# Project-MONAI/GenerativeModels

Hardware: NVIDIA H100
Metric: ddim50_voxels_per_s (higher is better)
Workload: dtype fp16

## Files before the change

generativemodels_b200/_lib.py:

```python
from __future__ import annotations

import ctypes as C
import os
from pathlib import Path

_HERE = Path(__file__).resolve().parent
ACT_DTYPE = os.environ.get("B200_ACT_DTYPE", "fp16").lower()
if ACT_DTYPE in ("float16", "half", "f16"):
    ACT_DTYPE = "fp16"
if ACT_DTYPE in ("bfloat16",):
    ACT_DTYPE = "bf16"
if ACT_DTYPE not in ("fp16", "bf16"):
    raise ValueError(f"B200_ACT_DTYPE must be fp16 or bf16, got {ACT_DTYPE!r}")
LIB_PATH = _HERE / "lib" / ("libb200gen.so" if ACT_DTYPE == "fp16" else "libb200gen_bf16.so")

B200_OK, B200_EINVAL, B200_ENOTSUP, B200_ECUDA, B200_ENODEV = 0, -1, -2, -3, -4
DT_H16, DT_F32 = 0, 1
DT_F64, DT_FP16, DT_BF16 = 2, 3, 4
SSIM_MAX_K, SSIM_MAX_SCALES = 128, 32
H16_FP16, H16_BF16 = 0, 1
ACT_NONE, ACT_RELU, ACT_SILU, ACT_LEAKYRELU, ACT_GELU, ACT_TANH, ACT_SIGMOID = 0, 1, 2, 3, 4, 5, 6
ACT_GEGLU = 7
ACT_LEAKYRELU02 = 8
INTERP_BILINEAR, INTERP_BICUBIC = 0, 1
POOL_AVG, POOL_MAX = 0, 1
(INTERPOLATE_NEAREST, INTERPOLATE_LINEAR, INTERPOLATE_BILINEAR, INTERPOLATE_BICUBIC, INTERPOLATE_TRILINEAR,
 INTERPOLATE_AREA) = 0, 1, 2, 3, 4, 5
PRED_EPSILON, PRED_SAMPLE, PRED_V = 0, 1, 2
IGEMM_MAX_SEG = 128


class B200Error(RuntimeError):
    pass


class IgemmSeg(C.Structure):
    _fields_ = [("src", C.c_int8), ("dw", C.c_int8), ("dh", C.c_int8), ("dd", C.c_int8),
                ("c0", C.c_uint16), ("nchunks", C.c_uint16)]


class IgemmParams(C.Structure):
    _fields_ = [
        ("a_ptr", C.c_void_p * 2), ("a_C", C.c_int32 * 2), ("a_pitch", C.c_int32 * 2),
        ("in_N", C.c_int32), ("in_D", C.c_int32), ("in_H", C.c_int32), ("in_W", C.c_int32),
        ("stride_d", C.c_int32), ("stride_h", C.c_int32), ("stride_w", C.c_int32),
        ("w_ptr", C.c_void_p), ("w_rows", C.c_int32), ("w_pitch", C.c_int32), ("w_K", C.c_int32),
        ("w_bstride", C.c_int64), ("w_batched", C.c_int32), ("n_seg", C.c_int32),
        ("seg", IgemmSeg * IGEMM_MAX_SEG),
        ("out_ptr", C.c_void_p), ("out_dtype", C.c_int32),
        ("out_N", C.c_int32), ("out_D", C.c_int32), ("out_H", C.c_int32), ("out_W", C.c_int32),
        ("cout", C.c_int32), ("out_cols", C.c_int32),
        ("out_sN", C.c_int64), ("out_sD", C.c_int64), ("out_sH", C.c_int64), ("out_sW", C.c_int64),
        ("bias", C.c_void_p), ("rowvec", C.c_void_p), ("rowvec_bstride", C.c_int64), ("row_bias", C.c_void_p),
        ("act1", C.c_int32), ("scale", C.c_float),
        ("res_ptr", C.c_void_p), ("res_dtype", C.c_int32),
        ("res_sN", C.c_int64), ("res_sD", C.c_int64), ("res_sH", C.c_int64), ("res_sW", C.c_int64),
        ("act2", C.c_int32), ("stat_ptr", C.c_void_p), ("impl", C.c_int32),
        ("gn_partial", C.c_void_p), ("gn_slots", C.c_int32), ("gn_slot0", C.c_int32),
        ("split_ws", C.c_void_p), ("split_ws_bytes", C.c_int64),
        ("a_broadcast", C.c_int32), ("gn_group", C.c_int32),
    ]


class GnStatsParams(C.Structure):
    _fields_ = [("x_ptr", C.c_void_p * 2), ("x_C", C.c_int32 * 2), ("x_pitch", C.c_int32 * 2),
                ("N", C.c_int32), ("spatial", C.c_int64), ("groups", C.c_int32), ("eps", C.c_float),
                ("gamma", C.c_void_p), ("beta", C.c_void_p), ("partial", C.c_void_p), ("affine", C.c_void_p)]


class GnApplyParams(C.Structure):
    _fields_ = [("x_ptr", C.c_void_p * 2), ("x_C", C.c_int32 * 2), ("x_pitch", C.c_int32 * 2),
                ("N", C.c_int32), ("spatial", C.c_int64), ("affine", C.c_void_p), ("act", C.c_int32),
                ("y_ptr", C.c_void_p), ("y_pitch", C.c_int32)]


class FlashParams(C.Structure):
    _fields_ = [("q", C.c_void_p), ("k", C.c_void_p), ("vt", C.c_void_p), ("out", C.c_void_p), ("res", C.c_void_p),
                ("B", C.c_int32), ("T", C.c_int32), ("S", C.c_int32), ("heads", C.c_int32), ("dh", C.c_int32),
                ("q_pitch", C.c_int32), ("k_pitch", C.c_int32), ("vt_pitch", C.c_int32), ("out_pitch", C.c_int32),
                ("res_pitch", C.c_int32), ("scale", C.c_float),
                ("workspace", C.c_void_p), ("workspace_bytes", C.c_int64)]


class DdimCoef(C.Structure):
    _fields_ = [("sqrt_alpha_prod_t", C.c_float), ("sqrt_beta_prod_t", C.c_float),
                ("sqrt_alpha_prod_prev", C.c_float), ("dir_coef", C.c_float), ("sigma", C.c_float),
                ("clip_min", C.c_float), ("clip_max", C.c_float),
                ("prediction_type", C.c_int32), ("clip", C.c_int32)]


class DdpmCoef(C.Structure):
    _fields_ = [("sqrt_alpha_prod_t", C.c_float), ("sqrt_beta_prod_t", C.c_float),
                ("coef_x0", C.c_float), ("coef_xt", C.c_float), ("sigma", C.c_float),
                ("clip_min", C.c_float), ("clip_max", C.c_float), ("min_log", C.c_float), ("max_log", C.c_float),
                ("var_mode", C.c_int32), ("prediction_type", C.c_int32), ("clip", C.c_int32)]

# ... 156 lines not shown
```

generativemodels_b200/csrc/igemm.cu:

```cuda
#include "common.cuh"
#include "wgmma.cuh"
#include <cuda.h>
#include <cudaTypedefs.h>
#include <mutex>
#include <string.h>

namespace b200 {

static constexpr int kBM = 128;
static constexpr int kBK = 64;
static constexpr int kABytes = kBM * kBK * 2;
static constexpr int kMmaWarp0 = 4;
static constexpr int kTmaWarp = 12;
static constexpr int kThreads = 13 * 32;

struct SegDev {
  int8_t src, dw, dh, dd;
  uint16_t c0, nchunks;
};

struct IgemmDev {
  alignas(64) CUtensorMap tmA[2];
  alignas(64) CUtensorMap tmB;
  const h16* a_ptr[2];
  int a_C[2], a_pitch[2];
  int in_N, in_D, in_H, in_W;
  int a_bcast;
  const h16* w_ptr;
  int w_rows, w_K, w_pitch;
  long long w_bstride;
  int w_batched;
  int n_seg, num_k_chunks;
  int sd, sh, sw;
  int N, OD, OH, OW;
  int BW, BH, BD, bw_log2, bh_log2;
  int tiles_w, tiles_h, tiles_d, tiles_n, num_tiles;
  int k_splits;
  long long split_stride;
  void* out_ptr;
  int out_dtype, cout, out_cols, out_vec, out_staged, out_v256;
  float* stat_ptr;
  float* gn_partial;
  int gn_slots, gn_slot0;
  int gn_sh;
  long long out_sN, out_sD, out_sH, out_sW;
  const float* bias;
  const float* rowvec;
  long long rowvec_bstride;
  const float* row_bias;
  int act1, act2;
  int geglu;
  float scale;
  const void* res_ptr;
  int res_dtype, res_vec, res_v256;
  long long res_sN, res_sD, res_sH, res_sW;
  SegDev seg[B200_IGEMM_MAX_SEG];
};

__device__ __forceinline__ void tma_load_5d(const CUtensorMap* tm, uint32_t bar, uint32_t dst, int c0,
                                            int c1, int c2, int c3, int c4) {
  asm volatile(
      "cp.async.bulk.tensor.5d.shared::cluster.global.mbarrier::complete_tx::bytes"
      " [%0], [%1, {%3, %4, %5, %6, %7}], [%2];" ::"r"(dst),
      "l"(reinterpret_cast<uint64_t>(tm)), "r"(bar), "r"(c0), "r"(c1), "r"(c2), "r"(c3), "r"(c4)
      : "memory");
}
template <int CH>
__device__ __forceinline__ void acc_ld(const float* src, uint32_t* r) {
#pragma unroll
  for (int j = 0; j < CH; j += 4) {
    const float4 t = *reinterpret_cast<const float4*>(src + j);
    r[j] = __float_as_uint(t.x); r[j + 1] = __float_as_uint(t.y);
    r[j + 2] = __float_as_uint(t.z); r[j + 3] = __float_as_uint(t.w);
  }
}

__host__ __device__ __forceinline__ int split_begin(int num_k, int splits, int ks) {
  return (int)(((long long)num_k * ks) / splits);
// ... 1145 lines not shown
  B200_CUDA(rc);
  if (max_clusters < 1) { set_error("igemm: no cluster of igemm_wide_kernel fits on this device"); return B200_ECUDA; }
  const int clusters = d.num_tiles < max_clusters ? d.num_tiles : max_clusters;
  B200_CUDA(b200::launch_kernel<wide::kCluster>(igemm_wide_kernel, clusters * wide::kCluster, wide::kThreads,
                                                wide::kSmem, stream, d));
  B200_LAUNCH_CHECK("igemm_wide_kernel");
  return B200_OK;
}

}

using namespace b200;

extern "C" int64_t b200_igemm_split_workspace_bytes(const b200_igemm_params* p) {
  if (!p || p->n_seg < 1 || p->n_seg > B200_IGEMM_MAX_SEG || p->out_N < 1 || p->out_D < 1 || p->out_H < 1 ||
      p->out_W < 1 || p->out_cols < 1 || p->stride_d < 1 || p->stride_h < 1 || p->stride_w < 1)
    return 0;
  if (p->impl == 1) return 0;
  return make_plan(p, true).ws_bytes;
}

extern "C" int b200_igemm_plan(const b200_igemm_params* p, int32_t sm_count_, int32_t with_workspace, int32_t out[4]) {
  if (!p || !out || sm_count_ < 1 || p->n_seg < 1 || p->n_seg > B200_IGEMM_MAX_SEG || p->out_N < 1 || p->out_D < 1 ||
      p->out_H < 1 || p->out_W < 1 || p->out_cols < 1)
    return B200_EINVAL;
  const Plan pl = make_plan(p, with_workspace != 0, sm_count_);
  out[0] = pl.BN;
  out[1] = pl.splits;
  out[2] = (int32_t)pl.ntiles;
  out[3] = 0;
  return B200_OK;
}

extern "C" int b200_igemm(const b200_igemm_params* p, void* stream_v) {
  cudaStream_t stream = static_cast<cudaStream_t>(stream_v);
  B200_CHECK_ARG(p != nullptr, "igemm: null params");
  B200_CHECK_ARG(p->a_ptr[0] && p->w_ptr && p->out_ptr, "igemm: null tensor pointer");
  B200_CHECK_ARG(p->n_seg >= 1 && p->n_seg <= B200_IGEMM_MAX_SEG, "igemm: n_seg=%d out of range", p->n_seg);
  B200_CHECK_ARG(p->in_N >= 1 && p->in_D >= 1 && p->in_H >= 1 && p->in_W >= 1, "igemm: bad input extent");
  B200_CHECK_ARG(p->out_N == p->in_N && p->out_D >= 1 && p->out_H >= 1 && p->out_W >= 1, "igemm: bad output extent");
  const bool geglu = p->act1 == B200_ACT_GEGLU;
  B200_CHECK_ARG(p->cout >= 1 && p->out_cols >= (geglu ? p->cout / 2 : p->cout), "igemm: bad cout/out_cols");
  if (geglu) {
    B200_CHECK_ARG(p->cout % 64 == 0 && p->out_cols == p->cout / 2 && p->out_dtype == B200_DT_H16 && !p->res_ptr &&
                   p->scale == 1.0f && p->act2 == B200_ACT_NONE && !p->stat_ptr && !p->gn_partial && !p->row_bias &&
                   p->impl != 1,
                   "igemm: B200_ACT_GEGLU needs cout %% 64 == 0, out_cols == cout / 2, a h16 output and no residual / "
                   "scale / act2 / statistics / row bias (and has no cross-check kernel)");
  }
  B200_CHECK_ARG(p->w_pitch % 8 == 0 && p->w_rows >= 1, "igemm: weight pitch must be a multiple of 8");
  B200_CHECK_ARG(((uintptr_t)p->w_ptr & 15) == 0, "igemm: weight pointer not 16-byte aligned");
  B200_CHECK_ARG(p->stride_d >= 1 && p->stride_d <= 8 && p->stride_h >= 1 && p->stride_h <= 8 &&
                 p->stride_w >= 1 && p->stride_w <= 8, "igemm: stride out of range");
  for (int s = 0; s < 2; ++s) {
    if (!p->a_ptr[s]) continue;
    B200_CHECK_ARG(p->a_pitch[s] % 8 == 0 && p->a_C[s] >= 1 && p->a_C[s] <= p->a_pitch[s],
                   "igemm: source %d channel pitch %d / extent %d invalid", s, p->a_pitch[s], p->a_C[s]);
    B200_CHECK_ARG(((uintptr_t)p->a_ptr[s] & 15) == 0, "igemm: source %d not 16-byte aligned", s);
  }
  std::call_once(g_encode_once, load_encode);
  if (!g_encode) { set_error("igemm: cuTensorMapEncodeTiled entry point unavailable"); return B200_ECUDA; }

  IgemmDev d;
  memset(&d, 0, sizeof(d));
  int kchunks = 0;
  for (int s = 0; s < p->n_seg; ++s) {
    const b200_igemm_seg& sg = p->seg[s];
    B200_CHECK_ARG(sg.src == 0 || (sg.src == 1 && p->a_ptr[1]), "igemm: segment %d uses missing source", s);
    B200_CHECK_ARG(sg.nchunks >= 1, "igemm: segment %d has no chunks", s);
    d.seg[s].src = sg.src; d.seg[s].dw = sg.dw; d.seg[s].dh = sg.dh; d.seg[s].dd = sg.dd;
    d.seg[s].c0 = sg.c0; d.seg[s].nchunks = sg.nchunks;
    kchunks += sg.nchunks;
  }
  const int w_K = p->w_K > 0 ? p->w_K : p->w_pitch;
  B200_CHECK_ARG(w_K <= p->w_pitch, "igemm: w_K %d exceeds the row pitch %d", w_K, p->w_pitch);
  d.n_seg = p->n_seg;
  d.num_k_chunks = kchunks;
  for (int s = 0; s < 2; ++s) {
    d.a_ptr[s] = reinterpret_cast<const h16*>(p->a_ptr[s]);
    d.a_C[s] = p->a_C[s];
    d.a_pitch[s] = p->a_pitch[s];
  }
  d.in_N = p->in_N; d.in_D = p->in_D; d.in_H = p->in_H; d.in_W = p->in_W;
  d.a_bcast = p->a_broadcast ? 1 : 0;
  d.w_ptr = reinterpret_cast<const h16*>(p->w_ptr);
  d.w_rows = p->w_rows; d.w_K = w_K; d.w_pitch = p->w_pitch;
  d.w_bstride = p->w_bstride; d.w_batched = p->w_batched;
  d.sd = p->stride_d; d.sh = p->stride_h; d.sw = p->stride_w;
  d.N = p->out_N; d.OD = p->out_D; d.OH = p->out_H; d.OW = p->out_W;
  d.out_ptr = p->out_ptr; d.out_dtype = p->out_dtype; d.cout = p->cout; d.out_cols = p->out_cols;
  d.out_sN = p->out_sN; d.out_sD = p->out_sD; d.out_sH = p->out_sH; d.out_sW = p->out_sW;
  d.bias = p->bias; d.rowvec = p->rowvec; d.rowvec_bstride = p->rowvec_bstride; d.row_bias = p->row_bias;
  d.act1 = geglu ? B200_ACT_NONE : p->act1; d.act2 = p->act2; d.scale = p->scale;
  d.geglu = geglu ? 1 : 0;
  if (geglu) d.out_cols = p->cout;
  d.res_ptr = p->res_ptr; d.res_dtype = p->res_dtype;
  d.res_sN = p->res_sN; d.res_sD = p->res_sD; d.res_sH = p->res_sH; d.res_sW = p->res_sW;
  {
    const int g = (p->out_dtype == B200_DT_H16) ? 8 : 4;
    d.out_vec = (p->out_cols % g == 0) && (p->out_sN % g == 0) && (p->out_sD % g == 0) &&
                (p->out_sH % g == 0) && (p->out_sW % g == 0) && (((uintptr_t)p->out_ptr) % 16 == 0);
    d.out_v256 = d.out_vec && p->out_dtype == B200_DT_H16 && (p->out_cols % 16 == 0) && (p->out_sN % 16 == 0) &&
                 (p->out_sD % 16 == 0) && (p->out_sH % 16 == 0) && (p->out_sW % 16 == 0) &&
                 (((uintptr_t)p->out_ptr) % 32 == 0);
  }
  B200_CHECK_ARG(!geglu || d.out_vec, "igemm: B200_ACT_GEGLU needs a 16-byte-aligned output (out_cols, strides %% 8 == 0)");
  {
    const long long esz = (p->out_dtype == B200_DT_H16) ? 2 : 4;
    d.out_staged = (p->out_sW * esz > 2048 && p->out_dtype == B200_DT_F32) ? 1 : 0;
  }
  d.gn_partial = p->gn_partial; d.gn_slots = p->gn_slots; d.gn_slot0 = p->gn_slot0;
  B200_CHECK_ARG(p->gn_group == 0 || p->gn_group == 8 || p->gn_group == 4, "igemm: gn_group must be 8 (or 0) or 4");
  d.gn_sh = (p->gn_group == 4) ? 2 : 3;
  if (p->gn_partial) {
    B200_CHECK_ARG(p->out_dtype == B200_DT_H16 && p->cout % 32 == 0 && d.out_vec && !d.out_staged && !p->stat_ptr && p->gn_slot0 >= 0 && p->gn_slot0 + 4 * sm_count() <= p->gn_slots,
                   "igemm: gn_partial needs an h16 vector-aligned output with cout %% 32 == 0 and 4 x SM-count slots");
  }
  d.stat_ptr = p->stat_ptr;
  if (p->stat_ptr)
    B200_CHECK_ARG(p->out_N == 1 && p->out_D == 1 && p->out_H == 1, "igemm: stat_ptr needs a GEMM-shaped call");
  if (p->res_ptr) {
    const int g = (p->res_dtype == B200_DT_H16) ? 8 : 4;
    d.res_vec = (p->out_cols % g == 0) && (p->res_sN % g == 0) && (p->res_sD % g == 0) &&
                (p->res_sH % g == 0) && (p->res_sW % g == 0) && (((uintptr_t)p->res_ptr) % 16 == 0);
    d.res_v256 = d.res_vec && p->res_dtype == B200_DT_H16 && (p->out_cols % 16 == 0) && (p->res_sN % 16 == 0) &&
                 (p->res_sD % 16 == 0) && (p->res_sH % 16 == 0) && (p->res_sW % 16 == 0) &&
                 (((uintptr_t)p->res_ptr) % 32 == 0);
    B200_CHECK_ARG(!p->gn_partial || (d.res_vec && p->res_dtype == B200_DT_H16),
                   "igemm: gn_partial needs a vector-aligned h16 residual");
  }

  const int impl = p->impl;
  B200_CHECK_ARG(impl >= 0 && impl <= 3, "igemm: impl %d not in 0..3", impl);
  B200_CHECK_ARG(impl != 1 || !p->stat_ptr, "igemm: stat_ptr has no cross-check kernel (impl 1)");
  B200_CHECK_ARG(impl != 3 || wide_fits(p),
                 "igemm: impl 3 (128 x 256 tiles) needs a vector-aligned h16 output with cout == out_cols a multiple of "
                 "256, a vector-aligned h16 residual or none, and no stat_ptr / GEGLU / row_bias / batched weights / "
                 "broadcast A");
  if (impl == 1) {
    const long long rows = (long long)d.N * d.OD * d.OH * d.OW;
    const long long total = rows * ((d.out_cols + 15) / 16);
    const int threads = 128;
    const long long blocks = (total + threads - 1) / threads;
    B200_CHECK_ARG(blocks < (1ll << 31), "igemm(check): problem too large");
    B200_CUDA(b200::launch_kernel(igemm_check_kernel, (unsigned)blocks, threads, 0, stream, d));
    B200_LAUNCH_CHECK("igemm_check_kernel");
    if (d.gn_partial) {
      const long long tot = rows * (d.cout >> d.gn_sh);
      B200_CUDA(b200::launch_kernel(gn8_partial_check_kernel, (unsigned)((tot + 255) / 256), 256, 0, stream, d));
      B200_LAUNCH_CHECK("gn8_partial_check_kernel");
    }
    return B200_OK;
  }

  const Plan pl = make_plan(p, p->split_ws != nullptr);
  const TileShape ts = pl.ts;
  d.BW = ts.bw; d.BH = ts.bh; d.BD = ts.bd;
  d.bw_log2 = ilog2(ts.bw); d.bh_log2 = ilog2(ts.bh);
  d.tiles_w = (d.OW + ts.bw - 1) / ts.bw;
  d.tiles_h = (d.OH + ts.bh - 1) / ts.bh;
  d.tiles_d = (d.OD + ts.bd - 1) / ts.bd;
  const int BN = pl.BN;
  d.tiles_n = pl.tiles_n;
  d.k_splits = 1;
  d.split_stride = 0;
  const int splits = (p->split_ws && pl.splits > 1) ? pl.splits : 1;
  if (splits > 1) {
    B200_CHECK_ARG(p->split_ws_bytes >= pl.ws_bytes && ((uintptr_t)p->split_ws & 15) == 0,
                   "igemm: split_ws needs %lld bytes, 16-byte aligned (got %lld)", pl.ws_bytes,
                   (long long)p->split_ws_bytes);
  }
  B200_CHECK_ARG(pl.ntiles * splits < (1ll << 31), "igemm: too many tiles");
  d.num_tiles = (int)pl.ntiles;

  for (int s = 0; s < 2; ++s) {
    if (!p->a_ptr[s]) continue;
    cuuint64_t dims[5] = {(cuuint64_t)p->a_C[s], (cuuint64_t)p->in_W, (cuuint64_t)p->in_H,
                          (cuuint64_t)p->in_D, (cuuint64_t)(p->a_broadcast ? 1 : p->in_N)};
    const cuuint64_t pb = (cuuint64_t)p->a_pitch[s] * 2;
    cuuint64_t strides[4] = {pb, pb * p->in_W, pb * p->in_W * p->in_H,
                             pb * p->in_W * p->in_H * p->in_D};
    cuuint32_t box[5] = {(cuuint32_t)kBK, (cuuint32_t)(ts.bw * d.sw), (cuuint32_t)(ts.bh * d.sh),
                         (cuuint32_t)(ts.bd * d.sd), 1};
    cuuint32_t estr[5] = {1, (cuuint32_t)d.sw, (cuuint32_t)d.sh, (cuuint32_t)d.sd, 1};
    CUresult r = g_encode(&d.tmA[s], B200_H16_TMAP, 5, const_cast<void*>(p->a_ptr[s]),
                          dims, strides, box, estr, CU_TENSOR_MAP_INTERLEAVE_NONE,
                          CU_TENSOR_MAP_SWIZZLE_128B, CU_TENSOR_MAP_L2_PROMOTION_L2_256B,
                          CU_TENSOR_MAP_FLOAT_OOB_FILL_NONE);
    if (r != CUDA_SUCCESS) {
      set_error("igemm: cuTensorMapEncodeTiled(A%d) failed with %d (C=%d pitch=%d in=%dx%dx%dx%d box=%ux%ux%u)",
                s, (int)r, p->a_C[s], p->a_pitch[s], p->in_N, p->in_D, p->in_H, p->in_W, box[1], box[2], box[3]);
      return B200_ECUDA;
    }
  }
  if (!p->a_ptr[1]) d.tmA[1] = d.tmA[0];
  {
    const int wbn = p->w_batched ? p->in_N : 1;
    cuuint64_t dims[3] = {(cuuint64_t)w_K, (cuuint64_t)p->w_rows, (cuuint64_t)wbn};
    cuuint64_t bs = p->w_bstride ? (cuuint64_t)p->w_bstride * 2 : (cuuint64_t)p->w_rows * p->w_pitch * 2;
    cuuint64_t strides[2] = {(cuuint64_t)p->w_pitch * 2, bs};
    B200_CHECK_ARG(bs % 16 == 0, "igemm: weight batch stride not 16-byte aligned");
    cuuint32_t box[3] = {(cuuint32_t)kBK, (cuuint32_t)(pl.wide ? 128 : BN), 1};
    cuuint32_t estr[3] = {1, 1, 1};
    CUresult r = g_encode(&d.tmB, B200_H16_TMAP, 3, const_cast<void*>(p->w_ptr), dims,
                          strides, box, estr, CU_TENSOR_MAP_INTERLEAVE_NONE, CU_TENSOR_MAP_SWIZZLE_128B,
                          CU_TENSOR_MAP_L2_PROMOTION_L2_256B, CU_TENSOR_MAP_FLOAT_OOB_FILL_NONE);
    if (r != CUDA_SUCCESS) {
      set_error("igemm: cuTensorMapEncodeTiled(W) failed with %d (K=%d rows=%d pitch=%d)", (int)r, w_K,
                p->w_rows, p->w_pitch);
      return B200_ECUDA;
    }
  }

  if (pl.wide) return launch_wide(d, stream);
  auto launch = [&](const IgemmDev& dev) {
    switch (BN) {
      case 16:  return launch_tc<16, 8>(dev, stream);
      case 32:  return launch_tc<32, 8>(dev, stream);
      case 64:  return launch_tc<64, 6>(dev, stream);
      default:  return launch_tc<128, 4>(dev, stream);
    }
  };
  if (splits == 1) return launch(d);

  IgemmDev ds = d;
  ds.k_splits = splits;
  ds.num_tiles = (int)(pl.ntiles * splits);
  ds.out_ptr = p->split_ws; ds.out_dtype = B200_DT_F32; ds.out_cols = pl.ws_cols;
  ds.out_sW = pl.ws_cols; ds.out_sH = ds.out_sW * d.OW; ds.out_sD = ds.out_sH * d.OH; ds.out_sN = ds.out_sD * d.OD;
  ds.split_stride = pl.rows * pl.ws_cols;
  ds.out_vec = 1; ds.out_v256 = 0;
  ds.out_staged = (ds.out_sW * 4 > 2048) ? 1 : 0;
  ds.bias = nullptr; ds.rowvec = nullptr; ds.row_bias = nullptr;
  ds.act1 = B200_ACT_NONE; ds.act2 = B200_ACT_NONE; ds.scale = 1.0f;
  ds.res_ptr = nullptr; ds.res_vec = 0; ds.res_v256 = 0;
  ds.stat_ptr = nullptr; ds.gn_partial = nullptr;
  const int rc = launch(ds);
  if (rc != B200_OK) return rc;
  const long long total = pl.rows * ((d.out_cols + 7) / 8);
  B200_CHECK_ARG((total + 255) / 256 < (1ll << 31), "igemm: split reduction too large");
  B200_CUDA(b200::launch_kernel(igemm_split_reduce_kernel, (unsigned)((total + 255) / 256), 256, 0, stream, 
      d, static_cast<const float*>(p->split_ws), splits, pl.ws_cols, ds.split_stride));
  B200_LAUNCH_CHECK("igemm_split_reduce_kernel");
  return B200_OK;
}
```

generativemodels_b200/networks/nets/diffusion_model_unet.py:

```python
from __future__ import annotations

import math
from collections.abc import Sequence

import torch
import torch.nn as nn

from ... import ops
from ...ops import ACT_SILU, CL
from ..blocks.spade_norm import SPADE
from .._holders import (Convolution, f32, on_input_device, packed_linear, packed_linear_geglu, packed_linear_stack,
                        require_cuda)

__all__ = ["DiffusionModelUNet"]


def zero_module(module: nn.Module) -> nn.Module:
    for p in module.parameters():
        p.detach().zero_()
    return module


def ensure_tuple_rep(v, n):
    if isinstance(v, (tuple, list)):
        if len(v) != n:
            raise ValueError(f"Sequence must have length {n}, got {len(v)}.")
        return tuple(v)
    return (v,) * n


def _rows(a: CL) -> torch.Tensor:
    return a.t.reshape(a.N, a.spatial, a.pitch)


def _context_cl(context: torch.Tensor) -> CL:
    return ops.to_cl(context.permute(0, 2, 1).unsqueeze(2).contiguous())


def _few_rows_linear(x: CL, pl) -> torch.Tensor:
    rows = x.N * x.spatial
    if rows <= 8 and x.C * rows * 2 <= 32 * 1024:
        y = ops.rows_linear(x.t.reshape(rows, x.pitch), x.C, pl)
        return y.reshape(x.N, x.spatial, y.shape[-1])
    return _rows(ops.linear(x, pl))


def _sdp(owner: nn.Module, xq: CL, xkv: CL, heads: int, dh: int, scale: float, residual: CL | None,
         bias_qkv: bool) -> CL:
    S = xkv.spatial
    inner = heads * dh
    use_tc = dh % 64 == 0 and S >= 64
    vt = vt_fork = None
    if use_tc:
        to_v = packed_linear(owner, "to_v")
        vt = ops.linear_transposed_out(_rows(xkv), to_v)
        with ops.fork() as vt_fork:
            ops.linear_transposed(_rows(xkv), xkv.C, to_v, out=vt)
    if xq is xkv and inner % 16 == 0:
        qk = ops.linear(xq, packed_linear_stack(owner, ("to_q", "to_k")))
        qk_rows = _rows(qk)
        q_rows, k_rows = qk_rows[:, :, :inner], qk_rows[:, :, inner:2 * inner]
    else:
        q_rows = _rows(ops.linear(xq, packed_linear(owner, "to_q")))
        k_rows = _few_rows_linear(xkv, packed_linear(owner, "to_k"))
    if use_tc:
# ... 139 lines not shown
        return self.op(x) if self.use_conv else ops.avgpool2(x)


class Upsample(nn.Module):

    def __init__(self, spatial_dims: int, num_channels: int, use_conv: bool, out_channels: int | None = None,
                 padding: int = 1) -> None:
        super().__init__()
        self.num_channels = num_channels
        self.out_channels = out_channels or num_channels
        self.use_conv = use_conv
        self.conv = Convolution(spatial_dims, self.num_channels, self.out_channels, strides=1, kernel_size=3,
                                padding=padding) if use_conv else None

    def forward(self, x: CL, emb=None) -> CL:
        if x.C != self.num_channels:
            raise ValueError("Input channels should be equal to num_channels")
        if self.use_conv:
            return self.conv.forward_upsampled(x)
        return ops.upsample_nearest2x(x)


class TimeEmb:

    __slots__ = ("emb", "proj")

    def __init__(self, emb: torch.Tensor, proj: dict) -> None:
        self.emb, self.proj = emb, proj


def project_time_embedding(root: nn.Module, emb: torch.Tensor) -> TimeEmb:
    blocks = root.__dict__.get("_temb_blocks")
    if blocks is None:
        blocks = root.__dict__["_temb_blocks"] = [m for m in root.modules() if isinstance(m, ResnetBlock)]
    if len(blocks) < 2:
        return TimeEmb(emb, {})
    params = []
    for b in blocks:
        params += [b.time_emb_proj.weight, b.time_emb_proj.bias]
    key = tuple((p.data_ptr(), p._version) for p in params)
    cache = root.__dict__.get("_temb_cat")
    if cache is None or cache[0] != key:
        w = torch.cat([b.time_emb_proj.weight.detach().float() for b in blocks], 0).contiguous()
        bias = torch.cat([b.time_emb_proj.bias.detach().float() for b in blocks], 0).contiguous()
        cache = root.__dict__["_temb_cat"] = (key, w, bias)
    rows = ops.small_linear(emb, cache[1], cache[2], act_in=ACT_SILU)
    proj, off = {}, 0
    for b in blocks:
        proj[id(b)] = rows[:, off:off + b.out_channels]
        off += b.out_channels
    return TimeEmb(emb, proj)


class ResnetBlock(nn.Module):

    def __init__(self, spatial_dims: int, in_channels: int, temb_channels: int, out_channels: int | None = None,
                 up: bool = False, down: bool = False, norm_num_groups: int = 32, norm_eps: float = 1e-6,
                 label_nc: int | None = None, spade_intermediate_channels: int = 128) -> None:
        super().__init__()
        self.spatial_dims = spatial_dims
        self.channels = in_channels
        self.emb_channels = temb_channels
        self.out_channels = out_channels or in_channels
        self.up, self.down = up, down
        self.spade = label_nc is not None

        def make_norm(ch):
            if self.spade:
                return SPADE(label_nc=label_nc, norm_nc=ch, norm="GROUP",
                             norm_params={"num_groups": norm_num_groups, "eps": norm_eps, "affine": True},
                             hidden_channels=spade_intermediate_channels, kernel_size=3, spatial_dims=spatial_dims)
            return nn.GroupNorm(num_groups=norm_num_groups, num_channels=ch, eps=norm_eps, affine=True)

        self.norm1 = make_norm(in_channels)
        self.nonlinearity = nn.SiLU()
        self.conv1 = Convolution(spatial_dims, in_channels, self.out_channels, strides=1, kernel_size=3, padding=1)
        self.upsample = self.downsample = None
        if self.up:
            self.upsample = Upsample(spatial_dims, in_channels, use_conv=False)
        elif down:
            self.downsample = Downsample(spatial_dims, in_channels, use_conv=False)
        self.time_emb_proj = nn.Linear(temb_channels, self.out_channels)
        self.norm2 = make_norm(self.out_channels)
        self.conv2 = zero_module(Convolution(spatial_dims, self.out_channels, self.out_channels, strides=1,
                                             kernel_size=3, padding=1))
        if self.out_channels == in_channels:
            self.skip_connection = nn.Identity()
        else:
            self.skip_connection = Convolution(spatial_dims, in_channels, self.out_channels, strides=1, kernel_size=1,
                                               padding=0)

    def _norm(self, norm, srcs, seg):
        if self.spade:
            if seg is None:
                raise ValueError("a SPADE ResnetBlock needs the segmentation map (seg)")
            return norm(srcs, seg, act=ACT_SILU)
        return ops.groupnorm(srcs, norm.num_groups, norm.eps, norm.weight, norm.bias, act=ACT_SILU)

    def forward(self, x: CL | Sequence[CL], emb: torch.Tensor, seg=None) -> CL:
        srcs = [x] if isinstance(x, CL) else list(x)
        h = self._norm(self.norm1, srcs, seg)
        if self.up or self.down:
            if len(srcs) != 1:
                raise ValueError("resampling ResnetBlock takes a single input tensor")
            resample = ops.upsample_nearest2x if self.up else ops.avgpool2
            srcs = [resample(srcs[0])]
            h = resample(h)
        skip_fork = None
        if isinstance(self.skip_connection, nn.Identity):
            skip = srcs[0] if len(srcs) == 1 else ops.concat(srcs)
        else:
            skip = self.skip_connection.empty_output(srcs)
            with ops.fork() as skip_fork:
                self.skip_connection(srcs, out=skip)
        temb = emb.proj.get(id(self)) if isinstance(emb, TimeEmb) else None
        if temb is None:
            e = emb.emb if isinstance(emb, TimeEmb) else emb
            temb = ops.small_linear(e, self.time_emb_proj.weight, self.time_emb_proj.bias, act_in=ACT_SILU)
        h = self.conv1(h, rowvec=temb)
        h = self._norm(self.norm2, [h], seg)
        if skip_fork is not None:
            skip_fork.join()
        return self.conv2(h, residual=skip)


def _downsampler(spatial_dims, out_channels, temb_channels, norm_num_groups, norm_eps, resblock_updown,
                 downsample_padding):
    if resblock_updown:
        return ResnetBlock(spatial_dims, out_channels, temb_channels, out_channels, down=True,
                           norm_num_groups=norm_num_groups, norm_eps=norm_eps)
    return Downsample(spatial_dims, out_channels, use_conv=True, out_channels=out_channels,
                      padding=downsample_padding)


def _upsampler(spatial_dims, out_channels, temb_channels, norm_num_groups, norm_eps, resblock_updown):
    if resblock_updown:
        return ResnetBlock(spatial_dims, out_channels, temb_channels, out_channels, up=True,
                           norm_num_groups=norm_num_groups, norm_eps=norm_eps)
    return Upsample(spatial_dims, out_channels, use_conv=True, out_channels=out_channels)


class _DownBase(nn.Module):

    def forward(self, hidden_states: CL, temb: torch.Tensor, context: CL | None = None):
        output_states = []
        attentions = self._modules.get("attentions")
        for i, resnet in enumerate(self.resnets):
            hidden_states = resnet(hidden_states, temb)
            if attentions is not None:
                attn = attentions[i]
                hidden_states = attn(hidden_states, context=context) if isinstance(attn, SpatialTransformer) \
                    else attn(hidden_states)
            output_states.append(hidden_states)
        if self.downsampler is not None:
            hidden_states = self.downsampler(hidden_states, temb)
            output_states.append(hidden_states)
        return hidden_states, output_states


class DownBlock(_DownBase):
    def __init__(self, spatial_dims: int, in_channels: int, out_channels: int, temb_channels: int,
                 num_res_blocks: int = 1, norm_num_groups: int = 32, norm_eps: float = 1e-6,
                 add_downsample: bool = True, resblock_updown: bool = False, downsample_padding: int = 1) -> None:
        super().__init__()
        self.resblock_updown = resblock_updown
        self.resnets = nn.ModuleList([
            ResnetBlock(spatial_dims, in_channels if i == 0 else out_channels, temb_channels, out_channels,
                        norm_num_groups=norm_num_groups, norm_eps=norm_eps) for i in range(num_res_blocks)])
        self.downsampler = _downsampler(spatial_dims, out_channels, temb_channels, norm_num_groups, norm_eps,
                                        resblock_updown, downsample_padding) if add_downsample else None

# ... 369 lines not shown
```

generativemodels_b200/ops.py:

```python
from __future__ import annotations

import ctypes as C
import numbers
import struct
import weakref
from dataclasses import dataclass
from typing import Sequence

import torch

from . import _lib
from ._lib import (ACT_GEGLU, ACT_GELU, ACT_LEAKYRELU, ACT_LEAKYRELU02, ACT_NONE, ACT_RELU, ACT_SIGMOID, ACT_SILU, ACT_TANH, DT_H16, DT_F32, DdimCoef, DdpmCoef, GnApplyParams, GnStatsParams,
                   IgemmParams, PndmCoef, check)

H16 = torch.float16 if _lib.ACT_DTYPE == "fp16" else torch.bfloat16

__all__ = ["CL", "to_cl", "from_cl", "PackedConv", "PackedConvTranspose", "PackedLinear", "conv", "conv_transpose",
           "linear", "linear_geglu", "fork", "groupnorm", "layernorm", "upsample_nearest2x", "avgpool2", "axpy", "geglu", "attention",
           "timestep_embedding", "small_linear", "ACT_NONE", "ACT_RELU", "ACT_SILU", "ACT_LEAKYRELU", "ACT_GELU", "ACT_TANH", "ACT_SIGMOID",
           "ACT_LEAKYRELU02", "upsample2x_interp", "vae_reparam_kld", "pool_s2", "batchnorm_fold", "interpolate",
           "interpolate_plan"]


def _stream() -> int:
# ... 97 lines not shown
    lib = _lib.require_device()
    N, D, H, W, P = t.shape
    shape = (N, C_, H, W) if spatial_dims == 2 else (N, C_, D, H, W)
    y = torch.empty(shape, dtype=torch.float32, device=t.device)
    check(lib.b200_nhwc_to_nchw(t.data_ptr(), DT_F32, N, C_, D * H * W, P, y.data_ptr(), _stream()), "b200_nhwc_to_nchw")
    return y


def _src_f32(weight: torch.Tensor) -> torch.Tensor:
    w = weight.detach()
    return w if (w.dtype == torch.float32 and w.is_contiguous()) else w.float().contiguous()


def repack(w: torch.Tensor, cout: int, cin: int, taps: int, blocks, rows: int, *, transposed: bool = False,
           mode: int = _lib.REPACK_BLOCKS, pitch: int | None = None) -> torch.Tensor:
    lib = _lib.require_device()
    arr, col = None, 0
    if mode == _lib.REPACK_BLOCKS:
        arr = (_lib.RepackBlock * len(blocks))()
        for i, (cin0, cs, taps_i) in enumerate(blocks):
            b = arr[i]
            b.col0, b.cin0, b.cs, b.ntaps = col, cin0, cs, len(taps_i)
            for j, t in enumerate(taps_i):
                b.tap[j] = t
            col += round_up(cs, 64)
        pitch = col
    out = torch.empty((round_up(rows, 16), pitch), dtype=H16, device=w.device)
    check(lib.b200_repack_weight(w.data_ptr(), cout, cin, taps, int(transposed), mode, arr, len(blocks) if blocks else 0,
                                 out.data_ptr(), out.shape[0], pitch, _stream()), "b200_repack_weight")
    return out


class PackedConv:

    def __init__(self, weight: torch.Tensor, bias: torch.Tensor | None, stride: int | Sequence[int],
                 padding, splits: Sequence[int] | None = None):
        w = _src_f32(weight)
        sd = w.dim() - 2
        self.spatial_dims = sd
        self.cout, cin = w.shape[0], w.shape[1]
        k = tuple(w.shape[2:])
        if sd == 2:
            k = (1, *k)
        self.k = k
        st = (stride,) * sd if isinstance(stride, int) else tuple(stride)
        self.stride = (1, *st) if sd == 2 else st
        if isinstance(padding, int):
            padding = [(padding, padding)] * sd
        padding = [(p, p) if isinstance(p, int) else tuple(p) for p in padding]
        self.pad = [(0, 0), *padding] if sd == 2 else padding
        self.splits = list(splits) if splits else [cin]
        if sum(self.splits) != cin or len(self.splits) > 2:
            raise ValueError(f"channel splits {self.splits} do not match weight in_channels {cin}")
        blocks, segs = [], []
        for a in range(k[0]):
            for b in range(k[1]):
                for c in range(k[2]):
                    off = 0
                    for s, cs in enumerate(self.splits):
                        blocks.append((off, cs, ((a * k[1] + b) * k[2] + c,)))
                        segs.append((s, c - self.pad[2][0], b - self.pad[1][0], a - self.pad[0][0], 0,
                                     round_up(cs, 64) // 64))
                        off += cs
        if len(segs) > _lib.IGEMM_MAX_SEG:
            raise ValueError(f"convolution needs {len(segs)} taps; the kernel supports {_lib.IGEMM_MAX_SEG}")
        taps = k[0] * k[1] * k[2]
        self.w = repack(w, self.cout, cin, taps, blocks, self.cout)
        self.segs = segs
        self.bias = None if bias is None else _src_f32(bias)
        self.tap_in = self.tap_out = None
        if taps > 1 and len(self.splits) == 1 and taps * cin <= 64:
            self.tap_in = PackedLinear.from_packed(repack(w, self.cout, cin, taps, None, self.cout,
                                                          mode=_lib.REPACK_TAP_IN, pitch=64),
                                                   self.cout, taps * cin, self.bias)
        elif (taps > 1 and len(self.splits) == 1 and self.cout <= 4 and taps * self.cout <= 128 and cin >= 64
              and self.stride == (1, 1, 1)):
            ncol = round_up(taps * self.cout, 32)
            self.tap_out = PackedLinear.from_packed(repack(w, self.cout, cin, taps, None, ncol,
                                                           mode=_lib.REPACK_TAP_OUT, pitch=round_up(cin, 64)),
                                                    ncol, cin, None)

    def geom(self, N: int, D: int, H: int, W: int):
        od = self.out_dims(D, H, W)
        return (C.c_int32 * 16)(N, D, H, W, *od, *self.k, *self.stride, self.pad[0][0], self.pad[1][0], self.pad[2][0])

    def out_dims(self, D: int, H: int, W: int) -> tuple[int, int, int]:
        i = (D, H, W)
        return tuple((i[d] + self.pad[d][0] + self.pad[d][1] - self.k[d]) // self.stride[d] + 1 for d in range(3))


class PackedLinear:

    def __init__(self, weight: torch.Tensor, bias: torch.Tensor | None):
        w = _src_f32(weight)
        self.cout, self.K = w.shape
        self.w = repack(w, self.cout, self.K, 1, [(0, self.K, (0,))], self.cout)
        self.segs = [(0, 0, 0, 0, 0, round_up(self.K, 64) // 64)]
        self.bias = None if bias is None else _src_f32(bias)
        self.stride = (1, 1, 1)

    @classmethod
    def stacked(cls, weights, biases) -> "PackedLinear":
        ws = [_src_f32(w) for w in weights]
        K = ws[0].shape[1]
        outs = [w.shape[0] for w in ws]
        if any(w.shape[1] != K for w in ws) or any(o % 16 for o in outs[:-1]):
            raise ValueError("stacked linears need a common input width and 16-row-aligned blocks")
        lib = _lib.require_device()
        pitch = round_up(K, 64)
        w16 = torch.empty((round_up(sum(outs), 16), pitch), dtype=H16, device=ws[0].device)
        blk = (_lib.RepackBlock * 1)()
        blk[0].col0, blk[0].cin0, blk[0].cs, blk[0].ntaps = 0, 0, K, 1
        row = 0
        for w, o in zip(ws, outs):
            rows_pad = round_up(o, 16)
            check(lib.b200_repack_weight(w.data_ptr(), o, K, 1, 0, _lib.REPACK_BLOCKS, blk, 1,
                                         w16.data_ptr() + row * pitch * 2, rows_pad, pitch, _stream()),
                  "b200_repack_weight")
            row += o
        bias = None
        if any(b is not None for b in biases):
            bias = torch.cat([(_src_f32(b) if b is not None else torch.zeros(o, device=ws[0].device))
                              for b, o in zip(biases, outs)]).contiguous()
        return cls.from_packed(w16, sum(outs), K, bias)

    @classmethod
    def geglu(cls, weight: torch.Tensor, bias: torch.Tensor | None) -> "PackedLinear":
        w = _src_f32(weight)
        H = w.shape[0] // 2
        if w.shape[0] != 2 * H or H % 32:
            raise ValueError(f"GEGLU linear needs 2 x (multiple of 32) output features, got {w.shape[0]}")
        j = torch.arange(2 * H, device=w.device)
        perm = (j // 64) * 32 + (j % 32) + ((j % 64) // 32) * H
# ... 161 lines not shown

def _conv_params(srcs: Sequence[CL], w: torch.Tensor, segs, stride, out_t: torch.Tensor, out_dims, cout: int,
                 out_dtype: int, bias, rowvec, act1: int, scale: float, res: torch.Tensor | None, res_dtype: int,
                 act2: int, out_elem_off: int = 0, out_strides=None, res_strides=None, impl: int = 0) -> IgemmParams:
    tmpl = _PARAM_TEMPLATES.get(id(w))
    if tmpl is not None and tmpl[0]() is w and tmpl[1] is segs:
        p = IgemmParams.from_buffer_copy(tmpl[2])
    else:
        p = IgemmParams()
        p.w_ptr = w.data_ptr()
        p.w_rows, p.w_pitch, p.w_K = w.shape[0], w.shape[1], 0
        p.w_bstride, p.w_batched = 0, 0
        _fill_segs(p, segs)
        if len(_PARAM_TEMPLATES) > 4096:
            _PARAM_TEMPLATES.clear()
        key = id(w)
        _PARAM_TEMPLATES[key] = (weakref.ref(w, lambda _r, _k=key: _PARAM_TEMPLATES.pop(_k, None)), segs,
                                 IgemmParams.from_buffer_copy(p))
    a0 = srcs[0]
    for i, a in enumerate(srcs):
        if (a.N, a.D, a.H, a.W) != (a0.N, a0.D, a0.H, a0.W):
            raise ValueError("concatenated inputs must share batch and spatial extent")
        p.a_ptr[i] = a.t.data_ptr()
        p.a_C[i] = a.C
        p.a_pitch[i] = a.pitch
    p.in_N, p.in_D, p.in_H, p.in_W = a0.N, a0.D, a0.H, a0.W
    p.stride_d, p.stride_h, p.stride_w = stride
    esz = 2 if out_dtype == DT_H16 else 4
    p.out_ptr = out_t.data_ptr() + out_elem_off * esz
    p.out_dtype = out_dtype
    p.out_N = a0.N
    p.out_D, p.out_H, p.out_W = out_dims
    P = out_t.shape[-1]
    p.cout, p.out_cols = cout, P
    if out_strides is None:
        OD, OH, OW = out_t.shape[1:4]
        out_strides = (OD * OH * OW * P, OH * OW * P, OW * P, P)
    p.out_sN, p.out_sD, p.out_sH, p.out_sW = out_strides
    p.bias = _ptr(bias)
    if rowvec is not None:
        p.rowvec = rowvec.data_ptr()
        p.rowvec_bstride = rowvec.stride(0) if rowvec.shape[0] > 1 else 0
    p.act1, p.scale, p.act2 = act1, scale, act2
    if res is not None:
        p.res_ptr = res.data_ptr() + (out_elem_off * (2 if res_dtype == DT_H16 else 4))
        p.res_dtype = res_dtype
        if res_strides is None:
            RP = res.shape[-1]
            RD, RH, RW = res.shape[1:4]
            res_strides = (RD * RH * RW * RP, RH * RW * RP, RW * RP, RP)
        p.res_sN, p.res_sD, p.res_sH, p.res_sW = res_strides
    p.impl = impl
    return p


def conv(srcs: CL | Sequence[CL], pc: PackedConv, *, rowvec: torch.Tensor | None = None, act1: int = ACT_NONE,
         scale: float = 1.0, residual: CL | None = None, act2: int = ACT_NONE, out_f32: bool = False,
         impl: int = 0, out: CL | None = None) -> CL | torch.Tensor:
    if isinstance(srcs, CL):
        srcs = [srcs]
    if [a.C for a in srcs] != pc.splits:
        raise ValueError(f"conv inputs have channels {[a.C for a in srcs]} but weights were packed for {pc.splits}")
    a0 = srcs[0]
    od = pc.out_dims(a0.D, a0.H, a0.W)
    if min(od) < 1:
        raise ValueError(f"convolution output would be empty for input {(a0.D, a0.H, a0.W)}")
    if out_f32:
        out_t = torch.empty((a0.N, *od, round_up(pc.cout, 4)), dtype=torch.float32, device=a0.t.device)
        out = out_t
    else:
        if out is None:
            out = new_cl(a0.N, od, pc.cout, a0.t.device, a0.spatial_dims)
        elif tuple(out.t.shape[:4]) != (a0.N, *od) or out.C != pc.cout:
            raise ValueError("preallocated convolution output has the wrong shape")
        out_t = out.t
    if residual is not None and tuple(residual.t.shape[:4]) != tuple(out_t.shape[:4]):
        raise ValueError("residual shape mismatch")
    rows = a0.N * od[0] * od[1] * od[2]
    if impl == 0 and rows >= _TAP_MIN_ROWS and pc.tap_in is not None:
        lib = _lib.require_device()
        Kp = round_up(pc.tap_in.K, 8)
        x2 = torch.empty((a0.N, *od, Kp), dtype=H16, device=a0.t.device)
        check(lib.b200_tap_gather(a0.t.data_ptr(), a0.C, a0.pitch, pc.geom(a0.N, a0.D, a0.H, a0.W), x2.data_ptr(), Kp,
                                  _stream()), "b200_tap_gather")
        pl = pc.tap_in
        p = _conv_params([CL(x2, pl.K, a0.spatial_dims)], pl.w, pl.segs, (1, 1, 1), out_t, od, pc.cout,
                         DT_F32 if out_f32 else DT_H16, pl.bias, rowvec, act1, scale,
                         None if residual is None else residual.t, DT_H16, act2)
        igemm_raw(p)
        return out
    if (impl == 0 and rows >= _TAP_MIN_ROWS and pc.tap_out is not None and rowvec is None and residual is None
            and act1 == ACT_NONE and act2 == ACT_NONE and scale == 1.0):
        lib = _lib.require_device()
        y = linear(a0, pc.tap_out, out_f32=True)
        check(lib.b200_tap_sum(y.data_ptr(), y.shape[-1], pc.geom(a0.N, a0.D, a0.H, a0.W), pc.cout, _ptr(pc.bias),
                               out_t.data_ptr(), out_t.shape[-1], DT_F32 if out_f32 else DT_H16, _stream()),
              "b200_tap_sum")
        return out
    p = _conv_params(srcs, pc.w, pc.segs, pc.stride, out_t, od, pc.cout, DT_F32 if out_f32 else DT_H16, pc.bias,
                     rowvec, act1, scale, None if residual is None else residual.t, DT_H16, act2, impl=impl)
    if not out_f32:
        part = _gn_partial_for(out, rows, len(pc.segs))
        if part is not None:
            p.gn_partial, p.gn_slots, p.gn_slot0 = part.data_ptr(), part.shape[1], 0
            p.gn_group = _gn_group(out)
    igemm_raw(p)
# ... 752 lines not shown
```

include/b200gen.h:

```cpp
#ifndef B200GEN_H_
#define B200GEN_H_

#include <stdint.h>

#ifdef __cplusplus
extern "C" {
#endif

#define B200_OK        0
#define B200_EINVAL   -1
#define B200_ENOTSUP  -2
#define B200_ECUDA    -3
#define B200_ENODEV   -4

#define B200_DT_H16  0
#define B200_DT_F32  1
#define B200_DT_F64  2
#define B200_DT_FP16 3
#define B200_DT_BF16 4
#define B200_H16_FP16 0
#define B200_H16_BF16 1

#define B200_ACT_NONE 0
#define B200_ACT_RELU 1
#define B200_ACT_SILU 2
#define B200_ACT_GELU 4
#define B200_ACT_TANH 5
#define B200_ACT_SIGMOID 6
#define B200_ACT_LEAKYRELU 3
#define B200_ACT_GEGLU 7
#define B200_ACT_LEAKYRELU02 8

#define B200_IGEMM_MAX_SEG 128

const char* b200_last_error_string(void);
int b200_version(void);
int b200_act_dtype(void);
int b200_device_check(void);
int b200_sm_count(void);
int b200_abi_sizeof(int which);

typedef struct {
  int8_t  src;
  int8_t  dw, dh, dd;
  uint16_t c0;
  uint16_t nchunks;
} b200_igemm_seg;

typedef struct {
  const void* a_ptr[2];
  int32_t a_C[2];
  int32_t a_pitch[2];
  int32_t in_N, in_D, in_H, in_W;
  int32_t stride_d, stride_h, stride_w;
  const void* w_ptr;
  int32_t w_rows;
  int32_t w_pitch;
  int32_t w_K;
  int64_t w_bstride;
  int32_t w_batched;
  int32_t n_seg;
  b200_igemm_seg seg[B200_IGEMM_MAX_SEG];
  void*   out_ptr;
  int32_t out_dtype;
  int32_t out_N, out_D, out_H, out_W;
  int32_t cout;
  int32_t out_cols;
  int64_t out_sN, out_sD, out_sH, out_sW;
  const float* bias;
  const float* rowvec;
  int64_t rowvec_bstride;
  const float* row_bias;
  int32_t act1;
  float   scale;
  const void* res_ptr;
  int32_t res_dtype;
  int64_t res_sN, res_sD, res_sH, res_sW;
  int32_t act2;
  float*  stat_ptr;
  int32_t impl;
  float*  gn_partial;
  int32_t gn_slots, gn_slot0;
  void*   split_ws;
  int64_t split_ws_bytes;
  int32_t a_broadcast;
  int32_t gn_group;
} b200_igemm_params;

int b200_igemm(const b200_igemm_params* p, void* stream);
int b200_igemm_plan(const b200_igemm_params* p, int32_t sm_count, int32_t with_workspace, int32_t out[4]);
int64_t b200_igemm_split_workspace_bytes(const b200_igemm_params* p);

typedef struct {
  const void* x_ptr[2];
  int32_t x_C[2];
  int32_t x_pitch[2];
  int32_t N;
  int64_t spatial;
  int32_t groups;
  float   eps;
  const float* gamma;
  const float* beta;
  float*  partial;
  float*  affine;
} b200_gn_stats_params;
// ... 171 lines not shown
```

Measured before the change: 146,500.

## Fold ResnetBlock skip connection into conv2 as extra K segments

Extends the implicit-GEMM conv kernel to accept up to three input sources. ResnetBlock can then fold its skip path (identity or 1x1 conv) into conv2 by appending the skip weights as extra K segments, and the skip bias is merged into the conv bias. This removes the separate skip conv launch or concat and the residual read in the epilogue. The trade-off is a longer K loop in conv2. The fold is gated by a plan check for the identity case and by a minimum row count for the 1x1 case.

```diff
diff --git a/generativemodels_b200/_lib.py b/generativemodels_b200/_lib.py
--- a/generativemodels_b200/_lib.py
+++ b/generativemodels_b200/_lib.py
@@ -28,6 +28,7 @@
  INTERPOLATE_AREA) = 0, 1, 2, 3, 4, 5
 PRED_EPSILON, PRED_SAMPLE, PRED_V = 0, 1, 2
 IGEMM_MAX_SEG = 128
+IGEMM_MAX_SRC = 3
 
 
 class B200Error(RuntimeError):
@@ -41,7 +42,8 @@
 
 class IgemmParams(C.Structure):
     _fields_ = [
-        ("a_ptr", C.c_void_p * 2), ("a_C", C.c_int32 * 2), ("a_pitch", C.c_int32 * 2),
+        ("a_ptr", C.c_void_p * IGEMM_MAX_SRC), ("a_C", C.c_int32 * IGEMM_MAX_SRC),
+        ("a_pitch", C.c_int32 * IGEMM_MAX_SRC),
         ("in_N", C.c_int32), ("in_D", C.c_int32), ("in_H", C.c_int32), ("in_W", C.c_int32),
         ("stride_d", C.c_int32), ("stride_h", C.c_int32), ("stride_w", C.c_int32),
         ("w_ptr", C.c_void_p), ("w_rows", C.c_int32), ("w_pitch", C.c_int32), ("w_K", C.c_int32),
diff --git a/generativemodels_b200/csrc/igemm.cu b/generativemodels_b200/csrc/igemm.cu
--- a/generativemodels_b200/csrc/igemm.cu
+++ b/generativemodels_b200/csrc/igemm.cu
@@ -20,10 +20,10 @@
 };
 
 struct IgemmDev {
-  alignas(64) CUtensorMap tmA[2];
+  alignas(64) CUtensorMap tmA[B200_IGEMM_MAX_SRC];
   alignas(64) CUtensorMap tmB;
-  const h16* a_ptr[2];
-  int a_C[2], a_pitch[2];
+  const h16* a_ptr[B200_IGEMM_MAX_SRC];
+  int a_C[B200_IGEMM_MAX_SRC], a_pitch[B200_IGEMM_MAX_SRC];
   int in_N, in_D, in_H, in_W;
   int a_bcast;
   const h16* w_ptr;
@@ -1275,7 +1275,7 @@
   B200_CHECK_ARG(((uintptr_t)p->w_ptr & 15) == 0, "igemm: weight pointer not 16-byte aligned");
   B200_CHECK_ARG(p->stride_d >= 1 && p->stride_d <= 8 && p->stride_h >= 1 && p->stride_h <= 8 &&
                  p->stride_w >= 1 && p->stride_w <= 8, "igemm: stride out of range");
-  for (int s = 0; s < 2; ++s) {
+  for (int s = 0; s < B200_IGEMM_MAX_SRC; ++s) {
     if (!p->a_ptr[s]) continue;
     B200_CHECK_ARG(p->a_pitch[s] % 8 == 0 && p->a_C[s] >= 1 && p->a_C[s] <= p->a_pitch[s],
                    "igemm: source %d channel pitch %d / extent %d invalid", s, p->a_pitch[s], p->a_C[s]);
@@ -1289,7 +1289,8 @@
   int kchunks = 0;
   for (int s = 0; s < p->n_seg; ++s) {
     const b200_igemm_seg& sg = p->seg[s];
-    B200_CHECK_ARG(sg.src == 0 || (sg.src == 1 && p->a_ptr[1]), "igemm: segment %d uses missing source", s);
+    B200_CHECK_ARG(sg.src >= 0 && sg.src < B200_IGEMM_MAX_SRC && p->a_ptr[sg.src],
+                   "igemm: segment %d uses missing source", s);
     B200_CHECK_ARG(sg.nchunks >= 1, "igemm: segment %d has no chunks", s);
     d.seg[s].src = sg.src; d.seg[s].dw = sg.dw; d.seg[s].dh = sg.dh; d.seg[s].dd = sg.dd;
     d.seg[s].c0 = sg.c0; d.seg[s].nchunks = sg.nchunks;
@@ -1299,7 +1300,7 @@
   B200_CHECK_ARG(w_K <= p->w_pitch, "igemm: w_K %d exceeds the row pitch %d", w_K, p->w_pitch);
   d.n_seg = p->n_seg;
   d.num_k_chunks = kchunks;
-  for (int s = 0; s < 2; ++s) {
+  for (int s = 0; s < B200_IGEMM_MAX_SRC; ++s) {
     d.a_ptr[s] = reinterpret_cast<const h16*>(p->a_ptr[s]);
     d.a_C[s] = p->a_C[s];
     d.a_pitch[s] = p->a_pitch[s];
@@ -1396,7 +1397,7 @@
   B200_CHECK_ARG(pl.ntiles * splits < (1ll << 31), "igemm: too many tiles");
   d.num_tiles = (int)pl.ntiles;
 
-  for (int s = 0; s < 2; ++s) {
+  for (int s = 0; s < B200_IGEMM_MAX_SRC; ++s) {
     if (!p->a_ptr[s]) continue;
     cuuint64_t dims[5] = {(cuuint64_t)p->a_C[s], (cuuint64_t)p->in_W, (cuuint64_t)p->in_H,
                           (cuuint64_t)p->in_D, (cuuint64_t)(p->a_broadcast ? 1 : p->in_N)};
@@ -1416,7 +1417,8 @@
       return B200_ECUDA;
     }
   }
-  if (!p->a_ptr[1]) d.tmA[1] = d.tmA[0];
+  for (int s = 1; s < B200_IGEMM_MAX_SRC; ++s)
+    if (!p->a_ptr[s]) d.tmA[s] = d.tmA[0];
   {
     const int wbn = p->w_batched ? p->in_N : 1;
     cuuint64_t dims[3] = {(cuuint64_t)w_K, (cuuint64_t)p->w_rows, (cuuint64_t)wbn};
diff --git a/generativemodels_b200/networks/nets/diffusion_model_unet.py b/generativemodels_b200/networks/nets/diffusion_model_unet.py
--- a/generativemodels_b200/networks/nets/diffusion_model_unet.py
+++ b/generativemodels_b200/networks/nets/diffusion_model_unet.py
@@ -9,8 +9,8 @@
 from ... import ops
 from ...ops import ACT_SILU, CL
 from ..blocks.spade_norm import SPADE
-from .._holders import (Convolution, f32, on_input_device, packed_linear, packed_linear_geglu, packed_linear_stack,
-                        require_cuda)
+from .._holders import (Convolution, _Cached, f32, on_input_device, packed_linear, packed_linear_geglu,
+                        packed_linear_stack, require_cuda)
 
 __all__ = ["DiffusionModelUNet"]
 
@@ -256,7 +256,10 @@
     return TimeEmb(emb, proj)
 
 
-class ResnetBlock(nn.Module):
+_FOLD_MIN_ROWS = 1 << 15
+
+
+class ResnetBlock(nn.Module, _Cached):
 
     def __init__(self, spatial_dims: int, in_channels: int, temb_channels: int, out_channels: int | None = None,
                  up: bool = False, down: bool = False, norm_num_groups: int = 32, norm_eps: float = 1e-6,
@@ -301,6 +304,27 @@
             return norm(srcs, seg, act=ACT_SILU)
         return ops.groupnorm(srcs, norm.num_groups, norm.eps, norm.weight, norm.bias, act=ACT_SILU)
 
+    def _folded_conv2(self, srcs: Sequence[CL]) -> ops.PackedConv | None:
+        a0, conv2 = srcs[0], self.conv2
+        splits = [a.C for a in srcs]
+        identity = isinstance(self.skip_connection, nn.Identity)
+        if identity:
+            k = (1, 3, 3) if self.spatial_dims == 2 else (3, 3, 3)
+            pad = [(0, 0), (1, 1), (1, 1)] if self.spatial_dims == 2 else [(1, 1)] * 3
+            dims = (a0.D, a0.H, a0.W)
+            _, segs = ops.PackedConv.tap_table(k, pad, [self.out_channels])
+            if not ops.plans_wide(segs, (1, 1, 1), self.out_channels, a0.N, dims, dims):
+                return None
+            params = (conv2.conv.weight, conv2.conv.bias)
+        else:
+            if a0.N * a0.D * a0.H * a0.W < _FOLD_MIN_ROWS:
+                return None
+            sk = self.skip_connection.conv
+            params = (conv2.conv.weight, conv2.conv.bias, sk.weight, sk.bias)
+        return self._cached(("conv2_skip", tuple(splits)), params, lambda: ops.PackedConv.with_skip(
+            conv2.conv.weight, conv2.conv.bias, conv2.padding, None if identity else params[2],
+            None if identity else params[3], splits))
+
     def forward(self, x: CL | Sequence[CL], emb: torch.Tensor, seg=None) -> CL:
         srcs = [x] if isinstance(x, CL) else list(x)
         h = self._norm(self.norm1, srcs, seg)
@@ -310,6 +334,15 @@
             resample = ops.upsample_nearest2x if self.up else ops.avgpool2
             srcs = [resample(srcs[0])]
             h = resample(h)
+        temb = emb.proj.get(id(self)) if isinstance(emb, TimeEmb) else None
+        if temb is None:
+            e = emb.emb if isinstance(emb, TimeEmb) else emb
+            temb = ops.small_linear(e, self.time_emb_proj.weight, self.time_emb_proj.bias, act_in=ACT_SILU)
+        folded = self._folded_conv2(srcs)
+        if folded is not None:
+            h = self.conv1(h, rowvec=temb)
+            h = self._norm(self.norm2, [h], seg)
+            return ops.conv([h, *srcs], folded)
         skip_fork = None
         if isinstance(self.skip_connection, nn.Identity):
             skip = srcs[0] if len(srcs) == 1 else ops.concat(srcs)
@@ -317,10 +350,6 @@
             skip = self.skip_connection.empty_output(srcs)
             with ops.fork() as skip_fork:
                 self.skip_connection(srcs, out=skip)
-        temb = emb.proj.get(id(self)) if isinstance(emb, TimeEmb) else None
-        if temb is None:
-            e = emb.emb if isinstance(emb, TimeEmb) else emb
-            temb = ops.small_linear(e, self.time_emb_proj.weight, self.time_emb_proj.bias, act_in=ACT_SILU)
         h = self.conv1(h, rowvec=temb)
         h = self._norm(self.norm2, [h], seg)
         if skip_fork is not None:
diff --git a/generativemodels_b200/ops.py b/generativemodels_b200/ops.py
--- a/generativemodels_b200/ops.py
+++ b/generativemodels_b200/ops.py
@@ -173,16 +173,7 @@
         self.splits = list(splits) if splits else [cin]
         if sum(self.splits) != cin or len(self.splits) > 2:
             raise ValueError(f"channel splits {self.splits} do not match weight in_channels {cin}")
-        blocks, segs = [], []
-        for a in range(k[0]):
-            for b in range(k[1]):
-                for c in range(k[2]):
-                    off = 0
-                    for s, cs in enumerate(self.splits):
-                        blocks.append((off, cs, ((a * k[1] + b) * k[2] + c,)))
-                        segs.append((s, c - self.pad[2][0], b - self.pad[1][0], a - self.pad[0][0], 0,
-                                     round_up(cs, 64) // 64))
-                        off += cs
+        blocks, segs = self.tap_table(k, self.pad, self.splits)
         if len(segs) > _lib.IGEMM_MAX_SEG:
             raise ValueError(f"convolution needs {len(segs)} taps; the kernel supports {_lib.IGEMM_MAX_SEG}")
         taps = k[0] * k[1] * k[2]
@@ -200,6 +191,51 @@
             self.tap_out = PackedLinear.from_packed(repack(w, self.cout, cin, taps, None, ncol,
                                                            mode=_lib.REPACK_TAP_OUT, pitch=round_up(cin, 64)),
                                                     ncol, cin, None)
+
+    @staticmethod
+    def tap_table(k, pad, splits):
+        blocks, segs = [], []
+        for a in range(k[0]):
+            for b in range(k[1]):
+                for c in range(k[2]):
+                    off = 0
+                    for s, cs in enumerate(splits):
+                        blocks.append((off, cs, ((a * k[1] + b) * k[2] + c,)))
+                        segs.append((s, c - pad[2][0], b - pad[1][0], a - pad[0][0], 0, round_up(cs, 64) // 64))
+                        off += cs
+        return blocks, segs
+
+    @classmethod
+    def with_skip(cls, weight: torch.Tensor, bias: torch.Tensor | None, padding, skip_weight: torch.Tensor | None,
+                  skip_bias: torch.Tensor | None, skip_splits: Sequence[int]) -> "PackedConv":
+        skip_splits = list(skip_splits)
+        if len(skip_splits) > _lib.IGEMM_MAX_SRC - 1:
+            raise ValueError(f"at most {_lib.IGEMM_MAX_SRC - 1} skip sources, got {skip_splits}")
+        self = cls(weight, None, 1, padding)
+        self.tap_in = self.tap_out = None
+        dev = self.w.device
+        if skip_weight is None:
+            if sum(skip_splits) != self.cout:
+                raise ValueError(f"an identity skip needs {self.cout} input channels, got {skip_splits}")
+            sw = torch.eye(self.cout, dtype=torch.float32, device=dev)
+        else:
+            sw = _src_f32(skip_weight).reshape(skip_weight.shape[0], -1)
+            if tuple(sw.shape) != (self.cout, sum(skip_splits)):
+                raise ValueError(f"1x1 skip weight {tuple(skip_weight.shape)} does not map {skip_splits} to "
+                                 f"{self.cout} channels")
+        blocks, off = [], 0
+        for cs in skip_splits:
+            blocks.append((off, cs, (0,)))
+            off += cs
+        self.w = torch.cat([self.w, repack(sw.contiguous(), self.cout, sw.shape[1], 1, blocks, self.cout)], 1)
+        self.segs = self.segs + [(1 + i, 0, 0, 0, 0, round_up(cs, 64) // 64) for i, cs in enumerate(skip_splits)]
+        if len(self.segs) > _lib.IGEMM_MAX_SEG:
+            raise ValueError(f"folded convolution needs {len(self.segs)} segments; the kernel supports "
+                             f"{_lib.IGEMM_MAX_SEG}")
+        self.splits = [self.splits[0], *skip_splits]
+        b = torch.zeros(self.cout, dtype=torch.float32, device=dev) if bias is None else _src_f32(bias)
+        self.bias = (b + _src_f32(skip_bias) if skip_bias is not None else b).contiguous()
+        return self
 
     def geom(self, N: int, D: int, H: int, W: int):
         od = self.out_dims(D, H, W)
@@ -467,6 +503,29 @@
         p.res_sN, p.res_sD, p.res_sH, p.res_sW = res_strides
     p.impl = impl
     return p
+
+
+_WIDE_PLANS: dict = {}
+
+
+def plans_wide(segs, stride, cout: int, N: int, in_dims: Sequence[int], out_dims: Sequence[int]) -> bool:
+    sm = int(_lib.require_device().b200_sm_count())
+    key = (tuple(segs), tuple(stride), cout, N, tuple(in_dims), tuple(out_dims), sm)
+    hit = _WIDE_PLANS.get(key)
+    if hit is None:
+        p = IgemmParams()
+        _fill_segs(p, segs)
+        p.in_N, (p.in_D, p.in_H, p.in_W) = N, in_dims
+        p.stride_d, p.stride_h, p.stride_w = stride
+        p.out_dtype, p.out_N, (p.out_D, p.out_H, p.out_W) = DT_H16, N, out_dims
+        P = round_up(cout, 8)
+        p.cout, p.out_cols = cout, P
+        OD, OH, OW = out_dims
+        p.out_sN, p.out_sD, p.out_sH, p.out_sW = OD * OH * OW * P, OH * OW * P, OW * P, P
+        out = (C.c_int32 * 4)()
+        check(_lib.load().b200_igemm_plan(C.byref(p), sm, 0, out), "b200_igemm_plan")
+        hit = _WIDE_PLANS[key] = out[0] == 256
+    return hit
 
 
 def conv(srcs: CL | Sequence[CL], pc: PackedConv, *, rowvec: torch.Tensor | None = None, act1: int = ACT_NONE,
diff --git a/include/b200gen.h b/include/b200gen.h
--- a/include/b200gen.h
+++ b/include/b200gen.h
@@ -32,6 +32,7 @@
 #define B200_ACT_LEAKYRELU02 8
 
 #define B200_IGEMM_MAX_SEG 128
+#define B200_IGEMM_MAX_SRC 3
 
 const char* b200_last_error_string(void);
 int b200_version(void);
@@ -48,9 +49,9 @@
 } b200_igemm_seg;
 
 typedef struct {
-  const void* a_ptr[2];
-  int32_t a_C[2];
-  int32_t a_pitch[2];
+  const void* a_ptr[B200_IGEMM_MAX_SRC];
+  int32_t a_C[B200_IGEMM_MAX_SRC];
+  int32_t a_pitch[B200_IGEMM_MAX_SRC];
   int32_t in_N, in_D, in_H, in_W;
   int32_t stride_d, stride_h, stride_w;
   const void* w_ptr;
```

Result: faster. 149,900, median of 6 (+2.3%).
